# csulb-datascience/TTS-with-Diffusion-model

Measured on AMD Instinct MI355X. Metric: EnCodec codec-tokens/sec (whole node), 100-step D3PM, higher is better.
Workload: dtype bf16; 1 GPU; libritts: d=512 H=8 L=6 T=750/768 S_text=50 S_prompt=225 99 diffusion iterations, n_q=1; utterances_per_gpu=32, global_batch=32, parallelism=dp1, streams_per_gpu=1

## Files before the change

tts-with-diffusion-model_amd/csrc/d3pm_api.hip:

```cpp
#include <cmath>
#include <cstdarg>
#include <cstdio>
#include <new>
#include <vector>

#include "d3pm_plan.h"

namespace d3pm {

static thread_local char g_err[512] = "";
void set_error(const char* fmt, ...) {
  va_list ap;
  va_start(ap, fmt);
  vsnprintf(g_err, sizeof(g_err), fmt, ap);
  va_end(ap);
}

int q_sample_launch(const d3pm_shape*, int, const int32_t*, int32_t*, const uint8_t*, int, const d3pm_schedule*,
                    uint64_t, uint32_t, hipStream_t);
int uniform_launch(uint64_t, int, uint32_t, int, int, int, float*, hipStream_t);
int ce_loss_launch(int, const void*, int, const int32_t*, const uint8_t*, int, int, int, float*, hipStream_t);
float host_h2f(uint16_t h);

}
// ... 940 lines not shown
                      void* workspace, size_t workspace_bytes, void* logits_out, void* hidden_out, int only_layers,
                      uint32_t flags, void* stream) {
  return denoise_step_impl(sh, w, batch, x_t, shared_mask(sh, frame_mask), t, film, kv_text, kv_prompt, workspace, workspace_bytes, logits_out,
                           hidden_out, only_layers, flags, stream, nullptr);
}

int d3pm_denoise_step_canvas(const d3pm_shape* sh, const d3pm_weights* w, int batch, const int32_t* x_t, const d3pm_canvas* canvas, int t,
                             const void* film, const void* kv_text, const void* kv_prompt, void* workspace, size_t workspace_bytes,
                             void* logits_out, void* hidden_out, int only_layers, uint32_t flags, void* stream) {
  D3PM_REQUIRE(canvas, D3PM_E_ARG, "d3pm_denoise_step_canvas: null canvas");
  return denoise_step_impl(sh, w, batch, x_t, per_utterance_mask(sh, batch, canvas, false), t, film, kv_text, kv_prompt, workspace, workspace_bytes,
                           logits_out, hidden_out, only_layers, flags, stream, nullptr);
}

int d3pm_denoise_step_keys(const d3pm_shape* sh, const d3pm_weights* w, int batch, const int32_t* x_t, const d3pm_canvas* canvas, int t,
                           const void* film, const void* kv_text, const void* kv_prompt, void* workspace, size_t workspace_bytes,
                           void* logits_out, void* hidden_out, int only_layers, uint32_t flags, const d3pm_keys* keys, void* stream) {
  D3PM_REQUIRE(canvas, D3PM_E_ARG, "d3pm_denoise_step_keys: null canvas");
  return denoise_step_impl(sh, w, batch, x_t, per_utterance_mask(sh, batch, canvas, false), t, film, kv_text, kv_prompt, workspace, workspace_bytes,
                           logits_out, hidden_out, only_layers, flags, stream, nullptr, key_counts(keys));
}

int d3pm_denoise_step_fp8(const d3pm_shape* sh, const d3pm_weights* w, const d3pm_fp8_block_weights* fp8_blocks, int batch,
                          const int32_t* x_t, const uint8_t* frame_mask, int t, const void* film, const void* kv_text,
                          const void* kv_prompt, void* workspace, size_t workspace_bytes, void* logits_out, void* hidden_out,
                          int only_layers, uint32_t flags, void* stream) {
  D3PM_REQUIRE(fp8_blocks, D3PM_E_ARG, "d3pm_denoise_step_fp8: null fp8 weights");
  return denoise_step_impl(sh, w, batch, x_t, shared_mask(sh, frame_mask), t, film, kv_text, kv_prompt, workspace, workspace_bytes, logits_out,
                           hidden_out, only_layers, flags, stream, fp8_blocks);
}

static int check_sampling(const d3pm_shape* sh, const d3pm_nucleus* sm, const char* who) {
  if (!sm) return D3PM_OK;
  D3PM_REQUIRE(std::isfinite(sm->temperature) && sm->temperature > 0.f, D3PM_E_ARG, "%s: temperature %g is not a finite number > 0", who,
               static_cast<double>(sm->temperature));
  D3PM_REQUIRE(sm->top_k >= 0 && sm->top_k <= sh->n_classes, D3PM_E_ARG, "%s: top_k %d outside 0 (off) .. %d (n_classes)", who, sm->top_k,
               sh->n_classes);
  D3PM_REQUIRE(std::isfinite(sm->top_p) && sm->top_p > 0.f && sm->top_p <= 1.f, D3PM_E_ARG, "%s: top_p %g outside (0, 1] (1 = off)", who,
               static_cast<double>(sm->top_p));
  return D3PM_OK;
}
static const d3pm_nucleus* with_top_p_off(const d3pm_sampling* sm, d3pm_nucleus* out) {
  if (!sm) return nullptr;
  *out = d3pm_nucleus{sm->temperature, sm->top_k, 1.0f};
  return out;
}

static int posterior_sample_impl(const d3pm_shape* sh, int batch, const void* logits, int logits_dtype, const int32_t* x_t,
                                 int32_t* x_next, const uint8_t* known, int t, const d3pm_schedule* sched, uint64_t seed, uint32_t utt0,
                                 uint32_t flags, uint16_t* posterior_out, void* stream, const d3pm_nucleus* sm = nullptr,
                                 float* theta_out = nullptr, const char* who = "d3pm_posterior_sample_sampling") {
  D3PM_TRY(check_shape(sh, batch));
  D3PM_TRY(check_sampling(sh, sm, who));
  D3PM_REQUIRE(logits && x_t && x_next && sched && sched->d && sched->c && sched->dbar && sched->cbar, D3PM_E_ARG,
               "d3pm_posterior_sample: null pointer");
  D3PM_REQUIRE(t >= 0 && t < sched->timesteps, D3PM_E_ARG, "t=%d outside the schedule", t);
  SampleArgs a;
  a.logits = logits; a.logits_dtype = logits_dtype; a.ldl = sh->n_classes; a.x_t = x_t; a.x_next = x_next;
  a.posterior_out = posterior_out; a.rows = batch * sh->canvas * levels(*sh); a.n_classes = sh->n_classes; a.mask_id = sh->mask_id;
  a.n_q = levels(*sh);
  a.canvas = sh->canvas; a.seed = seed; a.row0 = utt0 * static_cast<uint32_t>(sh->canvas);
  a.greedy = (flags & D3PM_FLAG_GREEDY) ? 1 : 0; a.pc = make_posterior_consts(sched, t);
  a.known = known;
  if (sm) { a.temperature = sm->temperature; a.top_k = sm->top_k; a.top_p = sm->top_p; }
  a.theta_out = theta_out;
  return posterior_sample(a, static_cast<hipStream_t>(stream));
}

int d3pm_posterior_sample(const d3pm_shape* sh, int batch, const void* logits, int logits_dtype, const int32_t* x_t,
                          int32_t* x_next, int t, const d3pm_schedule* sched, uint64_t seed, uint32_t utt0,
                          uint32_t flags, uint16_t* posterior_out, void* stream) {
  return posterior_sample_impl(sh, batch, logits, logits_dtype, x_t, x_next, nullptr, t, sched, seed, utt0, flags, posterior_out, stream);
}

int d3pm_posterior_sample_known(const d3pm_shape* sh, int batch, const void* logits, int logits_dtype, const int32_t* x_t,
                                int32_t* x_next, const uint8_t* known, int t, const d3pm_schedule* sched, uint64_t seed, uint32_t utt0,
                                uint32_t flags, uint16_t* posterior_out, void* stream) {
  return posterior_sample_impl(sh, batch, logits, logits_dtype, x_t, x_next, known, t, sched, seed, utt0, flags, posterior_out, stream);
}

int d3pm_posterior_sample_sampling(const d3pm_shape* sh, int batch, const void* logits, int logits_dtype, const int32_t* x_t,
                                   int32_t* x_next, const uint8_t* known, int t, const d3pm_schedule* sched, uint64_t seed, uint32_t utt0,
                                   uint32_t flags, uint16_t* posterior_out, const d3pm_sampling* sampling, void* stream) {
  d3pm_nucleus nu;
  return posterior_sample_impl(sh, batch, logits, logits_dtype, x_t, x_next, known, t, sched, seed, utt0, flags, posterior_out, stream,
                               with_top_p_off(sampling, &nu));
}

int d3pm_posterior_sample_nucleus(const d3pm_shape* sh, int batch, const void* logits, int logits_dtype, const int32_t* x_t,
                                  int32_t* x_next, const uint8_t* known, int t, const d3pm_schedule* sched, uint64_t seed, uint32_t utt0,
                                  uint32_t flags, uint16_t* posterior_out, const d3pm_nucleus* nucleus, float* theta_out, void* stream) {
  return posterior_sample_impl(sh, batch, logits, logits_dtype, x_t, x_next, known, t, sched, seed, utt0, flags, posterior_out, stream, nucleus,
                               theta_out, "d3pm_posterior_sample_nucleus");
}

int d3pm_op_posterior_sample_rows(const d3pm_shape* sh, int batch, const void* logits, int logits_dtype, int ldl, const int32_t* row_of,
                                  const int32_t* x_t, int32_t* x_next, int32_t* x_next2, const uint8_t* known, int t,
                                  const d3pm_schedule* sched, uint64_t seed, uint32_t utt0, uint32_t flags, const d3pm_nucleus* nucleus,
                                  const d3pm_guidance* guidance, void* stream) {
  const char* who = "d3pm_op_posterior_sample_rows";
  D3PM_TRY(check_shape(sh, batch));
  D3PM_TRY(check_sampling(sh, nucleus, who));
  D3PM_REQUIRE(logits && x_t && x_next && sched && sched->d && sched->c && sched->dbar && sched->cbar, D3PM_E_ARG, "%s: null pointer", who);
  D3PM_REQUIRE(t >= 0 && t < sched->timesteps, D3PM_E_ARG, "t=%d outside the schedule", t);
  D3PM_REQUIRE(ldl >= sh->n_classes, D3PM_E_ARG, "%s: row stride %d below n_classes %d", who, ldl, sh->n_classes);
  D3PM_REQUIRE(!(flags & D3PM_FLAG_SEED_IN_HBM), D3PM_E_ARG, "%s: the seed travels by value", who);
  SampleArgs a;
  a.logits = logits; a.logits_dtype = logits_dtype; a.ldl = ldl; a.x_t = x_t; a.x_next = x_next; a.x_next2 = x_next2;
  a.rows = batch * sh->canvas * levels(*sh); a.n_classes = sh->n_classes; a.mask_id = sh->mask_id; a.n_q = levels(*sh);
  a.canvas = sh->canvas; a.seed = seed; a.row0 = utt0 * static_cast<uint32_t>(sh->canvas);
  a.greedy = (flags & D3PM_FLAG_GREEDY) ? 1 : 0; a.pc = make_posterior_consts(sched, t);
  a.known = known;
  if (nucleus) { a.temperature = nucleus->temperature; a.top_k = nucleus->top_k; a.top_p = nucleus->top_p; }
  if (guidance) { a.guided = true; a.guidance = guidance->weight; }
  return posterior_sample_dedup(a, row_of, NextIterPrep{}, static_cast<hipStream_t>(stream));
}

static int sample_loop_impl(const d3pm_shape* sh, const d3pm_weights* w, int batch, int32_t* x, const CanvasMask& cm,
                            int t_start, int t_stop, const void* film, const void* kv_text, const void* kv_prompt,
                            const d3pm_schedule* sched, uint64_t seed, uint32_t utt0, uint32_t flags, void* workspace,
                            size_t workspace_bytes, int32_t* trace, void* stream, const d3pm_fp8_block_weights* f8,
                            const d3pm_nucleus* sm = nullptr, const char* who = "d3pm_sample_loop_sampling", const KeyCounts& keys = KeyCounts{},
                            const d3pm_guidance* guide = nullptr) {
  D3PM_TRY(check_shape(sh, batch));
  D3PM_TRY(check_sampling(sh, sm, who));
  D3PM_REQUIRE(w && w->blocks && x && cm.frame_mask && film && kv_text && kv_prompt && sched && workspace, D3PM_E_ARG,
               "d3pm_sample_loop: null pointer");
  D3PM_REQUIRE(t_start < sched->timesteps && t_start <= sh->timesteps && t_stop >= 0 && t_stop <= t_start, D3PM_E_ARG,
               "bad step range %d..%d", t_start, t_stop);
  d3pm_shape gsh;
  d3pm_tuning gtune;
  if (guide) {
    gtune = tune_of(sh->tuning);
    gtune.regime_batch = 2 * (gtune.regime_batch > batch ? gtune.regime_batch : batch);
    gsh = *sh;
    gsh.tuning = &gtune;
    sh = &gsh;
  }
  const int eval_batch = guide ? 2 * batch : batch;
  Workspace ws = carve(*sh, eval_batch, static_cast<char*>(workspace));
  D3PM_REQUIRE(workspace_bytes >= ws.total, D3PM_E_WORKSPACE, "workspace %zu < required %zu", workspace_bytes, ws.total);
  hipStream_t s = static_cast<hipStream_t>(stream);
  const int rows = batch * sh->canvas;
  const Ctx cx(sh->tuning);
  DenoiserArgs q{*sh, *w, eval_batch, cm.frame_mask, cm.period, kv_text, kv_prompt, ws, keys, guide ? rows : 0};
  const int plan = fold_plan(q, flags, f8);
  if (plan != FOLD_NONE && tune_of(sh->tuning).ln_fold != 2 && levels(*sh) == 1 && !guide && t_start - t_stop >= 2 && ws.tab_qkv) {
    D3PM_TRY(build_qkv_table(cx, *sh, *w, ws, s));
    q.qkv_table = ws.tab_qkv;
  }
  const int n_rows = eval_batch * sh->canvas;
  const int ln_fold = tune_of(sh->tuning).ln_fold;
  if (q.qkv_table && plan == FOLD_QUADS && (ln_fold == 1 || ln_fold == 4) && !f8 && !guide && ws.dd.row_of && n_rows % 384 == 0 && sh->n_layers <= 16 &&
      sh->n_classes <= kDedupMaxClasses && ws.h2 == at(ws.h, static_cast<size_t>(n_rows) * sh->d_model, dtype_size(sh->dtype))) {
    DedupPlanner dp{sh->dtype, sh->tuning, true};
    for (int l = 0; l < sh->n_layers; ++l) (void)folded_block(q, l, true, dp, l == 0);
    LinearArgs fin = projection(ws.x, w->final_w, w->final_b, ws.logits, n_rows, sh->n_classes, sh->d_model);
    fin.ldy = logits_ld(*sh); fin.tune = sh->tuning;
    const LinearPlan fp = plan_linear(sh->dtype, fin);
    const unsigned long long kv_rows = std::max<unsigned long long>(n_rows, qkv_table_rows(sh->n_classes));
    const bool gather_ok = static_cast<size_t>(sh->canvas) * 4 <= kGatherIndexBytes && kv_rows * 3 * sh->d_model * dtype_size(sh->dtype) < (1ull << 32);
    if (dp.ok && gather_ok && (fp.big() || fp.kernel == LIN_128_GLDS)) q.dd = &ws.dd;
  }
  bool latency_ok = false;
  if (q.dd && ln_fold == 1 && !cm.known) {
    DenoiserArgs ql = q;
    ql.m_est = live_latency_rows();
    DedupPlanner lp{sh->dtype, sh->tuning, true, LIN_PANEL64};
    for (int l = 0; l < sh->n_layers; ++l) (void)folded_block(ql, l, false, lp, l == 0);
    latency_ok = lp.ok;
  }
  auto latency_est = [&](int t) {
    if (!latency_ok || t <= t_stop) return 0;
    const int est = plan_live_rows(eval_batch, sh->canvas, host_h2f(sched->cbar[t]));
    return live_latency(est) ? est : 0;
  };
  bool prepared = false;
  bool qkv_ready = false;
  for (int t = t_start; t > t_stop; --t) {
    if (cx.prof) cx.prof->sample_now = (t % cx.prof->stride) == 0;
    q.m_est = latency_est(t);
    D3PM_TRY(denoiser_blocks(q, x, t, film, sh->n_layers, flags, s, f8, q.m_est ? FOLD_PARTS : plan, prepared, qkv_ready));
    prepared = qkv_ready = false;
    SampleArgs a;
    a.logits = ws.logits; a.logits_dtype = sh->dtype; a.ldl = logits_ld(*sh); a.x_t = x; a.x_next = x;
    a.x_next2 = trace ? trace + static_cast<size_t>(t_start - t) * rows * levels(*sh) : nullptr;
    a.rows = rows * levels(*sh); a.n_q = levels(*sh); a.n_classes = sh->n_classes; a.mask_id = sh->mask_id; a.canvas = sh->canvas; a.seed = seed;
    if (flags & D3PM_FLAG_SEED_IN_HBM) a.seed_hbm = reinterpret_cast<const uint64_t*>(static_cast<uintptr_t>(seed));
    a.row0 = utt0 * static_cast<uint32_t>(sh->canvas); a.greedy = (flags & D3PM_FLAG_GREEDY) ? 1 : 0;
    a.pc = make_posterior_consts(sched, t);
    a.known = cm.known;
    if (sm) { a.temperature = sm->temperature; a.top_k = sm->top_k; a.top_p = sm->top_p; }
    if (guide) { a.guided = true; a.guidance = guide->weight; }
    {
      D3PM_TRY(final_logits(*sh, *w, eval_batch, ws, ws.logits, logits_ld(*sh), flags, s, q.dd ? q.dd->m_live : nullptr));
      const bool preps = t - 1 > t_stop && plan != FOLD_NONE;
      if (q.dd) {
        NextIterPrep nx;
        if (preps) {
          nx.dtype = sh->dtype; nx.d = sh->d_model; nx.blocks = w->blocks; nx.n_layers = sh->n_layers;
          nx.film_t = at(film, static_cast<size_t>(t - 1) * sh->n_layers * 2 * sh->d_model, dtype_size(sh->dtype));
          nx.Wf = ws.fc1f; nx.s_out = ws.fc1f_s; nx.b_out = ws.fc1f_b;
        }
        {
          ProfScope p(cx, D3PM_K_SAMPLE, s, 0.0, static_cast<double>(rows) * (sh->n_classes * dtype_size(sh->dtype) + 8.0));
          D3PM_TRY(posterior_sample_dedup(a, q.dd->row_of, nx, s));
        }
        if (preps) {
          D3PM_TRY(run_dedup_index(q, x, plan == FOLD_QUADS && !latency_est(t - 1), s));
          prepared = qkv_ready = true;
        }
        continue;
      }
      ProfScope p(cx, D3PM_K_SAMPLE, s, 0.0,
                  static_cast<double>(rows) * levels(*sh) * ((guide ? 2.0 : 1.0) * sh->n_classes * dtype_size(sh->dtype) + 8.0) +
                      (preps && q.qkv_table ? static_cast<double>(rows) * 3.0 * sh->d_model * dtype_size(sh->dtype) : 0.0));
      NextIterPrep nx;
      if (preps) {
        const size_t es = dtype_size(sh->dtype);
        nx.dtype = sh->dtype; nx.table = w->resps_emb; nx.x = ws.x; nx.stats = ws.stats; nx.frame_mask = cm.frame_mask; nx.mask_period = cm.period; nx.d = sh->d_model;
        nx.quads = plan == FOLD_QUADS;
        nx.blocks = w->blocks; nx.n_layers = sh->n_layers;
        nx.film_t = at(film, static_cast<size_t>(t - 1) * sh->n_layers * 2 * sh->d_model, es);
        nx.Wf = ws.fc1f; nx.s_out = ws.fc1f_s; nx.b_out = ws.fc1f_b;
        if (q.qkv_table) { nx.qkv_table = q.qkv_table; nx.q0 = ws.q0; nx.kv0 = ws.kv0; }
      }
      if (nx.table && posterior_sample_prep_supported(a, nx)) {
        D3PM_TRY(guide ? posterior_sample_prep_guided(a, nx, s) : posterior_sample_prep(a, nx, s));
        prepared = true;
        qkv_ready = nx.q0 != nullptr;
      } else {
        D3PM_TRY(guide ? posterior_sample_guided(a, s) : posterior_sample(a, s));
      }
    }
  }
  if (cx.prof) cx.prof->sample_now = false;
  return D3PM_OK;
}

int d3pm_sample_loop(const d3pm_shape* sh, const d3pm_weights* w, int batch, int32_t* x, const uint8_t* frame_mask,
                     int t_start, int t_stop, const void* film, const void* kv_text, const void* kv_prompt,
                     const d3pm_schedule* sched, uint64_t seed, uint32_t utt0, uint32_t flags, void* workspace,
                     size_t workspace_bytes, int32_t* trace, void* stream) {
  return sample_loop_impl(sh, w, batch, x, shared_mask(sh, frame_mask), t_start, t_stop, film, kv_text, kv_prompt, sched, seed, utt0, flags,
                          workspace, workspace_bytes, trace, stream, nullptr);
}

int d3pm_sample_loop_canvas(const d3pm_shape* sh, const d3pm_weights* w, int batch, int32_t* x, const d3pm_canvas* canvas,
                            int t_start, int t_stop, const void* film, const void* kv_text, const void* kv_prompt,
                            const d3pm_schedule* sched, uint64_t seed, uint32_t utt0, uint32_t flags, void* workspace,
                            size_t workspace_bytes, int32_t* trace, void* stream) {
  D3PM_REQUIRE(canvas, D3PM_E_ARG, "d3pm_sample_loop_canvas: null canvas");
  return sample_loop_impl(sh, w, batch, x, per_utterance_mask(sh, batch, canvas, true), t_start, t_stop, film, kv_text, kv_prompt, sched, seed,
                          utt0, flags, workspace, workspace_bytes, trace, stream, nullptr);
}

int d3pm_sample_loop_fp8(const d3pm_shape* sh, const d3pm_weights* w, const d3pm_fp8_block_weights* fp8_blocks, int batch,
                         int32_t* x, const uint8_t* frame_mask, int t_start, int t_stop, const void* film,
                         const void* kv_text, const void* kv_prompt, const d3pm_schedule* sched, uint64_t seed, uint32_t utt0,
                         uint32_t flags, void* workspace, size_t workspace_bytes, int32_t* trace, void* stream) {
  D3PM_REQUIRE(fp8_blocks, D3PM_E_ARG, "d3pm_sample_loop_fp8: null fp8 weights");
  return sample_loop_impl(sh, w, batch, x, shared_mask(sh, frame_mask), t_start, t_stop, film, kv_text, kv_prompt, sched, seed, utt0, flags,
                          workspace, workspace_bytes, trace, stream, fp8_blocks);
}

int d3pm_sample_loop_fp8_canvas(const d3pm_shape* sh, const d3pm_weights* w, const d3pm_fp8_block_weights* fp8_blocks, int batch,
                                int32_t* x, const d3pm_canvas* canvas, int t_start, int t_stop, const void* film,
                                const void* kv_text, const void* kv_prompt, const d3pm_schedule* sched, uint64_t seed, uint32_t utt0,
                                uint32_t flags, void* workspace, size_t workspace_bytes, int32_t* trace, void* stream) {
  D3PM_REQUIRE(fp8_blocks && canvas, D3PM_E_ARG, "d3pm_sample_loop_fp8_canvas: null fp8 weights or canvas");
  return sample_loop_impl(sh, w, batch, x, per_utterance_mask(sh, batch, canvas, true), t_start, t_stop, film, kv_text, kv_prompt, sched, seed,
                          utt0, flags, workspace, workspace_bytes, trace, stream, fp8_blocks);
}

int d3pm_sample_loop_sampling(const d3pm_shape* sh, const d3pm_weights* w, const d3pm_fp8_block_weights* fp8_blocks, int batch, int32_t* x,
                              const uint8_t* frame_mask, const d3pm_canvas* canvas, int t_start, int t_stop, const void* film,
                              const void* kv_text, const void* kv_prompt, const d3pm_schedule* sched, uint64_t seed, uint32_t utt0,
                              uint32_t flags, void* workspace, size_t workspace_bytes, int32_t* trace, const d3pm_sampling* sampling,
                              void* stream) {
  D3PM_REQUIRE(sh && (frame_mask != nullptr) != (canvas != nullptr), D3PM_E_ARG,
               "d3pm_sample_loop_sampling: give exactly one of frame_mask (shared by the batch) and canvas (per utterance)");
  d3pm_nucleus nu;
  return sample_loop_impl(sh, w, batch, x, canvas ? per_utterance_mask(sh, batch, canvas, true) : shared_mask(sh, frame_mask), t_start, t_stop,
                          film, kv_text, kv_prompt, sched, seed, utt0, flags, workspace, workspace_bytes, trace, stream, fp8_blocks,
                          with_top_p_off(sampling, &nu));
}

int d3pm_sample_loop_nucleus(const d3pm_shape* sh, const d3pm_weights* w, const d3pm_fp8_block_weights* fp8_blocks, int batch, int32_t* x,
                             const uint8_t* frame_mask, const d3pm_canvas* canvas, int t_start, int t_stop, const void* film,
                             const void* kv_text, const void* kv_prompt, const d3pm_schedule* sched, uint64_t seed, uint32_t utt0,
                             uint32_t flags, void* workspace, size_t workspace_bytes, int32_t* trace, const d3pm_nucleus* nucleus,
                             void* stream) {
  D3PM_REQUIRE(sh && (frame_mask != nullptr) != (canvas != nullptr), D3PM_E_ARG,
               "d3pm_sample_loop_nucleus: give exactly one of frame_mask (shared by the batch) and canvas (per utterance)");
  return sample_loop_impl(sh, w, batch, x, canvas ? per_utterance_mask(sh, batch, canvas, true) : shared_mask(sh, frame_mask), t_start, t_stop,
                          film, kv_text, kv_prompt, sched, seed, utt0, flags, workspace, workspace_bytes, trace, stream, fp8_blocks, nucleus,
                          "d3pm_sample_loop_nucleus");
}

int d3pm_sample_loop_keys(const d3pm_shape* sh, const d3pm_weights* w, const d3pm_fp8_block_weights* fp8_blocks, int batch, int32_t* x,
                          const uint8_t* frame_mask, const d3pm_canvas* canvas, int t_start, int t_stop, const void* film,
                          const void* kv_text, const void* kv_prompt, const d3pm_schedule* sched, uint64_t seed, uint32_t utt0,
                          uint32_t flags, void* workspace, size_t workspace_bytes, int32_t* trace, const d3pm_nucleus* nucleus,
                          const d3pm_keys* keys, void* stream) {
  D3PM_REQUIRE(sh && (frame_mask != nullptr) != (canvas != nullptr), D3PM_E_ARG,
               "d3pm_sample_loop_keys: give exactly one of frame_mask (shared by the batch) and canvas (per utterance)");
  D3PM_REQUIRE(!(keys && fp8_blocks), D3PM_E_ARG, "d3pm_sample_loop_keys: the fp8 fast path takes no key mask");
// ... 552 lines not shown
```

tts-with-diffusion-model_amd/csrc/d3pm_dedup.hip:

```cpp
#include <climits>

#include "d3pm_kernels.h"
#include "d3pm_fold_rows.h"

namespace d3pm {
namespace {

__device__ __forceinline__ int clamp_id(int id, int n_classes) { return id < 0 ? 0 : (id >= n_classes ? n_classes - 1 : id); }

__global__ __launch_bounds__(256) void dedup_index_utt(const int32_t* __restrict__ tokens, const uint8_t* __restrict__ frame_mask, int mask_period,
                                                       int canvas, int n_classes, int32_t* __restrict__ cnt, int32_t* __restrict__ row_of,
                                                       int32_t* __restrict__ rep_pos, int32_t* __restrict__ key_cls) {
  extern __shared__ int dedup_sm[];
  int* first = dedup_sm;
  int* rank = first + n_classes + 1;
  int* wsum = rank + n_classes + 1;
  const int b = blockIdx.x, tid = threadIdx.x, lane = tid & 63, wave = tid >> 6;
  const size_t row0 = static_cast<size_t>(b) * canvas;
  for (int c = tid; c <= n_classes; c += 256) first[c] = INT_MAX;
  __syncthreads();
  auto class_of = [&](int j) {
    const size_t r = row0 + j;
    return frame_mask[r % mask_period] ? clamp_id(tokens[r], n_classes) : n_classes;
  };
  for (int j = tid; j < canvas; j += 256) atomicMin(&first[class_of(j)], j);
  __syncthreads();
  int base = 0;
  for (int j0 = 0; j0 < canvas; j0 += 256) {
    const int j = j0 + tid;
    int c = 0;
    bool rep = false;
    if (j < canvas) { c = class_of(j); rep = first[c] == j; }
    const unsigned long long m = __ballot(rep);
    if (lane == 0) wsum[wave] = __popcll(m);
    __syncthreads();
    int off = base;
    for (int w = 0; w < wave; ++w) off += wsum[w];
    if (rep) {
      const int k = off + __popcll(m & ((1ull << lane) - 1ull));
      rank[c] = k;
      rep_pos[row0 + k] = j;
    }
    base += wsum[0] + wsum[1] + wsum[2] + wsum[3];
    __syncthreads();
  }
  for (int j = tid; j < canvas; j += 256) {
    const int c = class_of(j);
    row_of[row0 + j] = rank[c];
    if (key_cls) key_cls[row0 + j] = c;
  }
  if (tid == 0) cnt[b] = base;
}

template <typename T>
__global__ __launch_bounds__(256) void dedup_embed_rows(const int32_t* __restrict__ tokens, const uint8_t* __restrict__ frame_mask, int mask_period,
                                                        int batch, int canvas, int n_classes, int d, int seg_align, const int32_t* __restrict__ cnt,
                                                        int32_t* __restrict__ seg_start, int32_t* __restrict__ seg_len, int32_t* __restrict__ m_live_out,
                                                        int32_t* __restrict__ row_of, const int32_t* __restrict__ rep_pos, int32_t* __restrict__ cid,
                                                        uint8_t* __restrict__ cmask, const T* __restrict__ table, T* __restrict__ x,
                                                        float* __restrict__ stats, bool quads, const T* __restrict__ qkv_table, T* __restrict__ q0,
                                                        T* __restrict__ zero0, T* __restrict__ zero1) {
  const int wave = threadIdx.x >> 6, lane = threadIdx.x & 63;
  const int n = batch * canvas;
  const int r = blockIdx.x * 4 + wave;
  if (r >= n) return;
  const int ub = r / canvas;
  int start = 0, u = -1, u_start = 0, u_cnt = 0, pos_start = 0, own_start = 0, own_len = 0;
  for (int b = 0; b < batch; ++b) {
    const int c = cnt[b], pad = (c + seg_align - 1) & ~(seg_align - 1);
    if (r >= start && r < start + pad) { u = b; u_start = start; u_cnt = c; }
    if (b == ub) pos_start = start;
    if (b == r) { own_start = start; own_len = pad; }
    start += pad;
  }
  const int m_live = start, m_pad = (m_live + 383) / 384 * 384;
  if (lane == 0) {
    if (r < batch) { seg_start[r] = own_start; seg_len[r] = own_len; }
    if (r == 0) *m_live_out = m_live;
  }
  if (lane == 0) row_of[r] += pos_start;
  if (r >= m_pad) return;
  int id = 0;
  bool live = false;
  if (u >= 0 && r - u_start < u_cnt) {
    const size_t row = static_cast<size_t>(u) * canvas + rep_pos[static_cast<size_t>(u) * canvas + (r - u_start)];
    id = clamp_id(tokens[row], n_classes);
    live = frame_mask[row % mask_period] != 0;
  }
  if (table) embed_row_stats<T>(table, id, live, x, r, d, n_classes, stats, quads, lane);
  if (qkv_table) {
    const Vec8<T>* ts = reinterpret_cast<const Vec8<T>*>(qkv_table + static_cast<size_t>(live ? id : n_classes) * 3 * d);
    Vec8<T>* tq = reinterpret_cast<Vec8<T>*>(q0 + static_cast<size_t>(r) * d);
    for (int c = lane; c < (d >> 3); c += kWave) tq[c] = ts[c];
  }
  if (lane == 0) {
    cid[r] = live ? id : n_classes;
    cmask[r] = live ? 1 : 0;
  }
  if (r >= m_live) {
    if (zero0) { Vec8<T>* z = reinterpret_cast<Vec8<T>*>(zero0 + static_cast<size_t>(r) * d); for (int c = lane; c < (d >> 3); c += kWave) z[c] = Vec8<T>{}; }
    if (zero1) { Vec8<T>* z = reinterpret_cast<Vec8<T>*>(zero1 + static_cast<size_t>(r) * d); for (int c = lane; c < (d >> 3); c += kWave) z[c] = Vec8<T>{}; }
  }
}

}

int dedup_index(int dtype, const DedupArgs& a, hipStream_t s) {
  const DedupIndex& ix = a.ix;
  D3PM_REQUIRE(a.tokens && a.frame_mask && a.mask_period > 0 && a.batch > 0 && a.canvas > 0 && a.n_classes > 0 && ix.cnt && ix.seg_start && ix.seg_len &&
                   ix.m_live && ix.row_of && ix.rep_pos && ix.cid && ix.cmask,
               D3PM_E_ARG, "row deduplication: null pointer");
  D3PM_REQUIRE(a.seg_align == 1 || a.seg_align == 128, D3PM_E_ARG, "row deduplication: seg_align is 1 or 128, not %d", a.seg_align);
  D3PM_REQUIRE(a.n_classes <= kDedupMaxClasses && a.canvas % 128 == 0 && (static_cast<long long>(a.batch) * a.canvas) % 384 == 0, D3PM_E_SHAPE,
               "row deduplication: at most %d classes, canvas a multiple of 128 and batch * canvas a multiple of 384", kDedupMaxClasses);
  D3PM_REQUIRE((dtype == D3PM_F16 || dtype == D3PM_BF16) && a.d % 8 == 0 && (!a.quads || a.d == 512) && (!a.table || (a.x && a.stats)) &&
                   (a.qkv_table != nullptr) == (a.q0 != nullptr),
               D3PM_E_ARG, "row deduplication: bad embedding arguments");
  const int n = a.batch * a.canvas;
  const size_t lds = (2 * static_cast<size_t>(a.n_classes + 1) + 4) * sizeof(int);
  dedup_index_utt<<<dim3(a.batch), dim3(256), lds, s>>>(a.tokens, a.frame_mask, a.mask_period, a.canvas, a.n_classes, ix.cnt, ix.row_of, ix.rep_pos, ix.key_cls);
  D3PM_LAUNCH_CHECK();
  const dim3 grid(static_cast<unsigned>((n + 3) / 4)), block(256);
  auto go = [&](auto* tag) {
    using U = std::remove_pointer_t<decltype(tag)>;
    dedup_embed_rows<U><<<grid, block, 0, s>>>(a.tokens, a.frame_mask, a.mask_period, a.batch, a.canvas, a.n_classes, a.d, a.seg_align, ix.cnt, ix.seg_start,
                                               ix.seg_len, ix.m_live, ix.row_of, ix.rep_pos, ix.cid, ix.cmask, static_cast<const U*>(a.table), static_cast<U*>(a.x),
                                               a.stats, a.quads, static_cast<const U*>(a.qkv_table), static_cast<U*>(a.q0),
                                               static_cast<U*>(a.zero[0]), static_cast<U*>(a.zero[1]));
  };
  if (dtype == D3PM_F16) go(static_cast<f16*>(nullptr)); else go(static_cast<bf16*>(nullptr));
  D3PM_LAUNCH_CHECK();
  return D3PM_OK;
}

}
```

tts-with-diffusion-model_amd/csrc/d3pm_kernels.h:

```cpp
#pragma once
#include "d3pm_common.h"

namespace d3pm {

enum { ACT_NONE = 0, ACT_GELU = 1, ACT_RELU = 2, ACT_SILU = 3 };

inline const d3pm_tuning& tune_of(const d3pm_tuning* t) {
  static const d3pm_tuning kDefault = { 0,  1024,  0,  0,
                                        1,  1,  10,  1,
                                        0,  1,  nullptr};
  return t ? *t : kDefault;
}

struct LinearArgs {
  const void* X = nullptr; int ldx = 0;
  const void* W = nullptr;
  const void* bias = nullptr;
  void* Y = nullptr; int ldy = 0;
  const void* R1 = nullptr; const void* R2 = nullptr; int ldr = 0;
  const uint8_t* row_mask = nullptr; int mask_period = 1;
  int M = 0, N = 0, K = 0;
  int act = ACT_NONE;
  const d3pm_tuning* tune = nullptr;
  const float* fold_s = nullptr; const float* fold_b = nullptr; const float* stats_in = nullptr; float fold_eps = 1e-6f;
  float* stats_out = nullptr;
  bool moment_quads = false;
  const int* m_live = nullptr;
  int m_est = 0;
};
inline bool fold_args_ok(const LinearArgs& a) {
  auto al16 = [](const void* p) { return (reinterpret_cast<uintptr_t>(p) % 16) == 0; };
  if (a.fold_s) {
    if (!a.fold_b || !a.stats_in || a.R1 || a.row_mask || a.stats_out || (a.act != ACT_NONE && a.act != ACT_GELU)) return false;
    if (a.K % 256 != 0 || a.N % 4 != 0 || !al16(a.fold_s) || !al16(a.fold_b) || !al16(a.stats_in)) return false;
  } else if (a.fold_b || a.stats_in) {
    return false;
  }
  if (a.stats_out) {
    if (!a.R1 || a.act != ACT_NONE || a.N % 32 != 0 || (reinterpret_cast<uintptr_t>(a.stats_out) % 8) != 0) return false;
  }
  if (a.moment_quads) {
    if (!a.fold_s && !a.stats_out) return false;
    if ((a.fold_s && a.K != 512) || (a.stats_out && a.N != 512)) return false;
  }
  return true;
}

struct AttnArgs {
  const void* Q = nullptr; int ldq = 0;
  const void* K = nullptr; const void* V = nullptr; int ldkv = 0;
  void* O = nullptr; int ldo = 0;
  int B = 0, Tq = 0, S = 0, H = 0, hd = 0;
  float scale = 1.f;
  const int32_t* key_len = nullptr;
  const void* Q2 = nullptr; const void* K2 = nullptr; const void* V2 = nullptr; void* O2 = nullptr; int S2 = 0;
  const int32_t* key_len2 = nullptr;
  bool masked_keeps_schedule = false;
  const int32_t* seg_start = nullptr; const int32_t* seg_len = nullptr;
  const int32_t* key_row = nullptr; int kv_rows = 0;
  const d3pm_tuning* tune = nullptr;
};

struct LayerNormArgs {
  const void* X = nullptr; void* Y = nullptr;
  const void* w = nullptr; const void* b = nullptr;
  const void* w2 = nullptr; const void* b2 = nullptr; void* Y2 = nullptr;
  const void* film = nullptr;
  int M = 0, d = 0; float eps = 1e-6f;
  const int32_t* tokens = nullptr; const uint8_t* frame_mask = nullptr; int mask_period = 0, n_classes = 0; void* Xout = nullptr;
};

struct RowPanelFuse {
  const void* X2 = nullptr;
  const void* lnw = nullptr; const void* lnb = nullptr; void* lny = nullptr;
  const void* lnw2 = nullptr; const void* lnb2 = nullptr; void* lny2 = nullptr;
  const void* film = nullptr;
  float eps = 1e-6f;
  void* sx = nullptr; void* sx2 = nullptr;
};

struct EmbedArgs {
  const int32_t* tokens = nullptr; const uint8_t* frame_mask = nullptr; int mask_period = 0;
  const void* table = nullptr; void* Y = nullptr; int M = 0, d = 0, n_classes = 0;
  int n_q = 1;
  const void* qkv_table = nullptr; void* q0 = nullptr; void* kv0 = nullptr;
};
inline int qkv_table_rows(int n_classes) { return (n_classes + 1 + 383) / 384 * 384; }

struct PosteriorConsts {
  float log_f1_zero;
  float log_f1_d;
  float log_f1_c;
  float log_f1_one;
  float dbar_prev;
  float cbar_prev;
  int t;
};

struct SampleArgs {
  const void* logits = nullptr; int logits_dtype = D3PM_F16; int ldl = 0;
  const int32_t* x_t = nullptr; int32_t* x_next = nullptr; int32_t* x_next2 = nullptr;
  uint16_t* posterior_out = nullptr;
  int rows = 0, n_classes = 0, mask_id = 0, canvas = 0;
  uint64_t seed = 0; uint32_t row0 = 0; int greedy = 0;
  const uint64_t* seed_hbm = nullptr;
  int n_q = 1;
  const uint8_t* known = nullptr;
  float temperature = 1.0f; int top_k = 0;
  bool filtered() const { return temperature != 1.0f || top_k != 0; }
  float top_p = 1.0f; float* theta_out = nullptr;
  bool nucleus() const { return top_p < 1.0f || theta_out != nullptr; }
  bool guided = false; float guidance = 0.f;
  PosteriorConsts pc{};
};

int generic_linear(int dtype, const LinearArgs& a, hipStream_t s);
int generic_attention(int dtype, const AttnArgs& a, hipStream_t s);
struct DropoutArgs {
  float p = 0.f, s = 1.f;
  uint64_t seed = 0;
  uint32_t utt0 = 0, site = 0;
};
int generic_attention_dropout_f32(const AttnArgs& a, const DropoutArgs& dr, hipStream_t s);
int generic_layernorm(int dtype, const LayerNormArgs& a, hipStream_t s);
int embed_tokens(int dtype, const EmbedArgs& a, hipStream_t s);
int pad_heads(const void* in, void* out, long long rows, int groups, int hd, hipStream_t s);
int unpad_heads(const void* in, void* out, long long rows, int groups, int hd, hipStream_t s);
int cond_embed_text(int dtype, const int32_t* tok, const void* table, const void* pe0, void* y, int rows, int s_text, int d,
                    int n_classes, const int32_t* key_len, hipStream_t s);
int cond_embed_prompt(int dtype, const int32_t* codes, int n_levels, const void* tables, const void* pe, void* y,
                      int rows, int s_prompt, int d, int n_classes, const int32_t* key_len, hipStream_t s);
int posterior_sample(const SampleArgs& a, hipStream_t s);
struct NextIterPrep {
  int dtype = D3PM_BF16;
  const void* table = nullptr; void* x = nullptr; float* stats = nullptr; const uint8_t* frame_mask = nullptr; int d = 0;
  int mask_period = 0;
  bool quads = false;
  const d3pm_block_weights* blocks = nullptr; int n_layers = 0; const void* film_t = nullptr;
  void* Wf = nullptr; float* s_out = nullptr; float* b_out = nullptr;
  const void* qkv_table = nullptr; void* q0 = nullptr; void* kv0 = nullptr;
};
bool posterior_sample_prep_supported(const SampleArgs& a, const NextIterPrep& n);
int posterior_sample_prep(const SampleArgs& a, const NextIterPrep& n, hipStream_t s);
int posterior_sample_guided(const SampleArgs& a, hipStream_t s);

struct DedupIndex {
  int32_t* cnt = nullptr;
  int32_t* seg_start = nullptr;
  int32_t* seg_len = nullptr;
  int32_t* m_live = nullptr;
  int32_t* row_of = nullptr;
  int32_t* key_cls = nullptr;
  int32_t* rep_pos = nullptr;
  int32_t* cid = nullptr;
  uint8_t* cmask = nullptr;
};
struct DedupArgs {
  const int32_t* tokens = nullptr; const uint8_t* frame_mask = nullptr; int mask_period = 0;
  int batch = 0, canvas = 0, n_classes = 0, d = 0;
  DedupIndex ix;
  int seg_align = 128;
  const void* table = nullptr; void* x = nullptr; float* stats = nullptr; bool quads = false;
  const void* qkv_table = nullptr; void* q0 = nullptr;
  void* zero[2] = {nullptr, nullptr};
};
constexpr int kDedupMaxClasses = 4095;
int dedup_index(int dtype, const DedupArgs& a, hipStream_t s);
int posterior_sample_dedup(const SampleArgs& a, const int32_t* row_of, const NextIterPrep& n, hipStream_t s);
int posterior_sample_prep_guided(const SampleArgs& a, const NextIterPrep& n, hipStream_t s);

struct RevealArgs {
  const void* logits = nullptr; int logits_dtype = D3PM_F16; int ldl = 0;
  const int32_t* x_t = nullptr; int32_t* x_next = nullptr; int32_t* x_next2 = nullptr;
  const uint8_t* frame_mask = nullptr; int mask_period = 0;
  const uint8_t* known = nullptr;
  int32_t* cand = nullptr; float* score = nullptr;
  int rows = 0, canvas = 0, n_classes = 0, mask_id = 0;
  uint64_t seed = 0; uint32_t row0 = 0; int greedy = 0;
  int t = 0;
  float lambda = 0.f;
  float keep_frac = 0.f;
  float temperature = 1.0f; int top_k = 0; float top_p = 1.0f;
  bool filtered() const { return temperature != 1.0f || top_k != 0 || top_p < 1.0f; }
};
int reveal_candidates(const RevealArgs& a, hipStream_t s);
int reveal_commit(const RevealArgs& a, hipStream_t s);
bool reveal_commit_prep_supported(const RevealArgs& a, const NextIterPrep& n);
int reveal_commit_prep(const RevealArgs& a, const NextIterPrep& n, hipStream_t s);

struct MxLinearArgs {
  const void* X8 = nullptr; int ldx = 0; const void* SX = nullptr;
  const void* W8 = nullptr; const void* SW = nullptr;
  const void* bias = nullptr;
  void* Y = nullptr; int ldy = 0;
  const void* R1 = nullptr; int ldr = 0;
  const uint8_t* row_mask = nullptr; int mask_period = 1;
  void* Y8 = nullptr; void* SY = nullptr;
  int M = 0, N = 0, K = 0;
  int act = ACT_NONE;
  const d3pm_tuning* tune = nullptr;
};
bool mx_linear_supported(int dtype, const MxLinearArgs& a);
int mx_linear(int dtype, const MxLinearArgs& a, hipStream_t s);
int layernorm_mx(int dtype, const void* x, uint8_t* y8, uint8_t* sx, const void* w, const void* b, const void* film,
                 const void* w2, const void* b2, uint8_t* y8_2, uint8_t* sx_2, int M, int d, float eps, hipStream_t s);
int quantize_mx(int dtype, const void* x, int ldx, uint8_t* y8, uint8_t* sx, int M, int K, hipStream_t s);

struct LinearPlan;
struct AttnPlan;
int mfma_linear(int dtype, const LinearArgs& a, const LinearPlan& p, hipStream_t s);
int big_linear(int dtype, const LinearArgs& a, const LinearPlan& p, hipStream_t s);
int panel64_linear(int dtype, const LinearArgs& a, const LinearPlan& p, hipStream_t s);
int mfma_attention(int dtype, const AttnArgs& a, const AttnPlan& p, hipStream_t s);
int mfma_attention32(int dtype, const AttnArgs& a, const AttnPlan& p, hipStream_t s);
int mfma_attention32_cross(int dtype, const AttnArgs& a, const AttnPlan& p, hipStream_t s);
int mfma_attention_split(int dtype, const AttnArgs& a, const AttnPlan& p, hipStream_t s);
int panel64_dual(int dtype, const LinearArgs& a, const void* X2, const LinearPlan& p, hipStream_t s);
int big_dual(int dtype, const LinearArgs& a, const void* X2, const LinearPlan& p, hipStream_t s);
bool row_panel_supported(int dtype, const LinearArgs& a, const RowPanelFuse& f);
int row_panel_linear(int dtype, const LinearArgs& a, const RowPanelFuse& f, hipStream_t s);
bool fast_layernorm_supported(int dtype, const LayerNormArgs& a);
int fast_layernorm(int dtype, const LayerNormArgs& a, hipStream_t s);

PosteriorConsts make_posterior_consts(const d3pm_schedule* sched, int t);

bool fold_shape_ok(int dtype, int d);
int fold_rows_launch(int dtype, const void* W, const void* bias, const void* gamma, const void* beta, const void* film, long film_ld,
                     int n_rows, int n_t, int K, void* Wf, float* s_out, float* b_out, hipStream_t s);
int fold_fc1_step_launch(int dtype, const d3pm_block_weights* blocks, int n_layers, const void* film_t, int d, void* Wf, float* s_out,
                         float* b_out, hipStream_t s);
int row_stats_launch(int dtype, const void* x, int ldx, int M, int d, float* stats, hipStream_t s, bool quads = false);
int embed_tokens_stats(int dtype, const EmbedArgs& a, float* stats, bool quads, hipStream_t s);
int qkv_table_rows_launch(int dtype, const void* table, void* x, float* stats, int rows, int d, int n_classes, hipStream_t s);

struct NarEmbedArgs {
  const int32_t* lens = nullptr;
  const int32_t* text = nullptr; int tt_max = 0;
  const int32_t* prom = nullptr; int tp_max = 0; int n_prom_levels = 8;
  const int32_t* resp = nullptr; int tr_max = 0; int resp_stride = 8; int n_given = 1;
  const void *w_text = nullptr, *w_prom = nullptr, *w_resp = nullptr, *sep = nullptr, *pe = nullptr;
  void* x = nullptr; uint8_t* row_mask = nullptr; int32_t* key_len = nullptr;
  int batch = 0, t_max = 0, d = 0, n_tokens = 0;
};
int nar_embed(int dtype, const NarEmbedArgs& a, hipStream_t s);
int adaln(int dtype, const void* x, void* y, const void* emb_row, const uint8_t* row_mask, int M, int d, hipStream_t s);
int nar_sample(int dtype, const void* logits, int ldl, const int32_t* lens, int32_t* resp, int tr_max, int resp_stride,
               int t_max, int n_tokens, int level, float temperature, uint64_t seed, uint32_t utt0, int greedy, int batch,
               hipStream_t s);

}
```

Baseline: 204,600 codec_tokens/s.

## Compute dedup segment offsets once per block via scan and use persistent grid

The dedup embedding kernel used to loop over every utterance in each wave to find segment starts, one wave per row. It now computes the padded segment prefix sums once per block into LDS with a wave-shuffle scan, finds each row's utterance by binary search, and runs a fixed grid of 4 blocks per CU that loops over rows. This removes the redundant per-row O(batch) scan. In exchange it adds an LDS footprint that scales with batch, so a max-batch limit is enforced and the host plan falls back when eval_batch exceeds it.

```diff
diff --git a/tts-with-diffusion-model_amd/csrc/d3pm_api.hip b/tts-with-diffusion-model_amd/csrc/d3pm_api.hip
--- a/tts-with-diffusion-model_amd/csrc/d3pm_api.hip
+++ b/tts-with-diffusion-model_amd/csrc/d3pm_api.hip
@@ -1116,7 +1116,7 @@
   const int n_rows = eval_batch * sh->canvas;
   const int ln_fold = tune_of(sh->tuning).ln_fold;
   if (q.qkv_table && plan == FOLD_QUADS && (ln_fold == 1 || ln_fold == 4) && !f8 && !guide && ws.dd.row_of && n_rows % 384 == 0 && sh->n_layers <= 16 &&
-      sh->n_classes <= kDedupMaxClasses && ws.h2 == at(ws.h, static_cast<size_t>(n_rows) * sh->d_model, dtype_size(sh->dtype))) {
+      sh->n_classes <= kDedupMaxClasses && eval_batch <= kDedupMaxBatch && ws.h2 == at(ws.h, static_cast<size_t>(n_rows) * sh->d_model, dtype_size(sh->dtype))) {
     DedupPlanner dp{sh->dtype, sh->tuning, true};
     for (int l = 0; l < sh->n_layers; ++l) (void)folded_block(q, l, true, dp, l == 0);
     LinearArgs fin = projection(ws.x, w->final_w, w->final_b, ws.logits, n_rows, sh->n_classes, sh->d_model);
diff --git a/tts-with-diffusion-model_amd/csrc/d3pm_dedup.hip b/tts-with-diffusion-model_amd/csrc/d3pm_dedup.hip
--- a/tts-with-diffusion-model_amd/csrc/d3pm_dedup.hip
+++ b/tts-with-diffusion-model_amd/csrc/d3pm_dedup.hip
@@ -2,6 +2,7 @@
 
 #include "d3pm_kernels.h"
 #include "d3pm_fold_rows.h"
+#include "d3pm_plan.h"
 
 namespace d3pm {
 namespace {
@@ -52,6 +53,8 @@
   if (tid == 0) cnt[b] = base;
 }
 
+constexpr int kEmbedGrid = 4 * kCUs;
+
 template <typename T>
 __global__ __launch_bounds__(256) void dedup_embed_rows(const int32_t* __restrict__ tokens, const uint8_t* __restrict__ frame_mask, int mask_period,
                                                         int batch, int canvas, int n_classes, int d, int seg_align, const int32_t* __restrict__ cnt,
@@ -60,46 +63,72 @@
                                                         uint8_t* __restrict__ cmask, const T* __restrict__ table, T* __restrict__ x,
                                                         float* __restrict__ stats, bool quads, const T* __restrict__ qkv_table, T* __restrict__ q0,
                                                         T* __restrict__ zero0, T* __restrict__ zero1) {
-  const int wave = threadIdx.x >> 6, lane = threadIdx.x & 63;
+  extern __shared__ int embed_sm[];
+  int* start = embed_sm;
+  int* wsum = start + batch + 1;
+  const int tid = threadIdx.x, wave = tid >> 6, lane = tid & 63;
   const int n = batch * canvas;
-  const int r = blockIdx.x * 4 + wave;
-  if (r >= n) return;
-  const int ub = r / canvas;
-  int start = 0, u = -1, u_start = 0, u_cnt = 0, pos_start = 0, own_start = 0, own_len = 0;
-  for (int b = 0; b < batch; ++b) {
-    const int c = cnt[b], pad = (c + seg_align - 1) & ~(seg_align - 1);
-    if (r >= start && r < start + pad) { u = b; u_start = start; u_cnt = c; }
-    if (b == ub) pos_start = start;
-    if (b == r) { own_start = start; own_len = pad; }
-    start += pad;
+  int base = 0;
+  for (int b0 = 0; b0 < batch; b0 += 256) {
+    const int b = b0 + tid;
+    const int pad = b < batch ? (cnt[b] + seg_align - 1) & ~(seg_align - 1) : 0;
+    int v = pad;
+#pragma unroll
+    for (int off = 1; off < kWave; off <<= 1) {
+      const int o = __shfl_up(v, off, kWave);
+      if (lane >= off) v += o;
+    }
+    if (lane == kWave - 1) wsum[wave] = v;
+    __syncthreads();
+    int before = base;
+    for (int w = 0; w < wave; ++w) before += wsum[w];
+    if (b < batch) start[b] = before + v - pad;
+    base += wsum[0] + wsum[1] + wsum[2] + wsum[3];
+    __syncthreads();
   }
-  const int m_live = start, m_pad = (m_live + 383) / 384 * 384;
-  if (lane == 0) {
-    if (r < batch) { seg_start[r] = own_start; seg_len[r] = own_len; }
-    if (r == 0) *m_live_out = m_live;
+  if (tid == 0) start[batch] = base;
+  __syncthreads();
+  const int m_live = base, m_pad = (m_live + 383) / 384 * 384;
+  if (blockIdx.x == 0) {
+    for (int b = tid; b < batch; b += 256) { seg_start[b] = start[b]; seg_len[b] = start[b + 1] - start[b]; }
+    if (tid == 0) *m_live_out = m_live;
   }
-  if (lane == 0) row_of[r] += pos_start;
-  if (r >= m_pad) return;
-  int id = 0;
-  bool live = false;
-  if (u >= 0 && r - u_start < u_cnt) {
-    const size_t row = static_cast<size_t>(u) * canvas + rep_pos[static_cast<size_t>(u) * canvas + (r - u_start)];
-    id = clamp_id(tokens[row], n_classes);
-    live = frame_mask[row % mask_period] != 0;
+  const int gw = blockIdx.x * 4 + wave, waves = gridDim.x * 4;
+  for (int r0 = gw * kWave; r0 < n; r0 += waves * kWave) {
+    const int r = r0 + lane;
+    if (r < n) row_of[r] += start[r / canvas];
   }
-  if (table) embed_row_stats<T>(table, id, live, x, r, d, n_classes, stats, quads, lane);
-  if (qkv_table) {
-    const Vec8<T>* ts = reinterpret_cast<const Vec8<T>*>(qkv_table + static_cast<size_t>(live ? id : n_classes) * 3 * d);
-    Vec8<T>* tq = reinterpret_cast<Vec8<T>*>(q0 + static_cast<size_t>(r) * d);
-    for (int c = lane; c < (d >> 3); c += kWave) tq[c] = ts[c];
-  }
-  if (lane == 0) {
-    cid[r] = live ? id : n_classes;
-    cmask[r] = live ? 1 : 0;
-  }
-  if (r >= m_live) {
-    if (zero0) { Vec8<T>* z = reinterpret_cast<Vec8<T>*>(zero0 + static_cast<size_t>(r) * d); for (int c = lane; c < (d >> 3); c += kWave) z[c] = Vec8<T>{}; }
-    if (zero1) { Vec8<T>* z = reinterpret_cast<Vec8<T>*>(zero1 + static_cast<size_t>(r) * d); for (int c = lane; c < (d >> 3); c += kWave) z[c] = Vec8<T>{}; }
+  const int m_end = m_pad < n ? m_pad : n;
+  for (int r = gw; r < m_end; r += waves) {
+    int id = 0;
+    bool live = false;
+    if (r < m_live) {
+      int lo = 0, hi = batch - 1;
+      while (lo < hi) {
+        const int mid = (lo + hi + 1) >> 1;
+        if (start[mid] <= r) lo = mid; else hi = mid - 1;
+      }
+      const int u = lo, k = r - start[u];
+      if (k < cnt[u]) {
+        const size_t row = static_cast<size_t>(u) * canvas + rep_pos[static_cast<size_t>(u) * canvas + k];
+        id = clamp_id(tokens[row], n_classes);
+        live = frame_mask[row % mask_period] != 0;
+      }
+    }
+    if (table) embed_row_stats<T>(table, id, live, x, r, d, n_classes, stats, quads, lane);
+    if (qkv_table) {
+      const Vec8<T>* ts = reinterpret_cast<const Vec8<T>*>(qkv_table + static_cast<size_t>(live ? id : n_classes) * 3 * d);
+      Vec8<T>* tq = reinterpret_cast<Vec8<T>*>(q0 + static_cast<size_t>(r) * d);
+      for (int c = lane; c < (d >> 3); c += kWave) tq[c] = ts[c];
+    }
+    if (lane == 0) {
+      cid[r] = live ? id : n_classes;
+      cmask[r] = live ? 1 : 0;
+    }
+    if (r >= m_live) {
+      if (zero0) { Vec8<T>* z = reinterpret_cast<Vec8<T>*>(zero0 + static_cast<size_t>(r) * d); for (int c = lane; c < (d >> 3); c += kWave) z[c] = Vec8<T>{}; }
+      if (zero1) { Vec8<T>* z = reinterpret_cast<Vec8<T>*>(zero1 + static_cast<size_t>(r) * d); for (int c = lane; c < (d >> 3); c += kWave) z[c] = Vec8<T>{}; }
+    }
   }
 }
 
@@ -116,14 +145,15 @@
   D3PM_REQUIRE((dtype == D3PM_F16 || dtype == D3PM_BF16) && a.d % 8 == 0 && (!a.quads || a.d == 512) && (!a.table || (a.x && a.stats)) &&
                    (a.qkv_table != nullptr) == (a.q0 != nullptr),
                D3PM_E_ARG, "row deduplication: bad embedding arguments");
-  const int n = a.batch * a.canvas;
+  D3PM_REQUIRE(a.batch <= kDedupMaxBatch, D3PM_E_SHAPE, "row deduplication: at most %d utterances", kDedupMaxBatch);
   const size_t lds = (2 * static_cast<size_t>(a.n_classes + 1) + 4) * sizeof(int);
   dedup_index_utt<<<dim3(a.batch), dim3(256), lds, s>>>(a.tokens, a.frame_mask, a.mask_period, a.canvas, a.n_classes, ix.cnt, ix.row_of, ix.rep_pos, ix.key_cls);
   D3PM_LAUNCH_CHECK();
-  const dim3 grid(static_cast<unsigned>((n + 3) / 4)), block(256);
+  const dim3 grid(kEmbedGrid), block(256);
+  const size_t embed_lds = (static_cast<size_t>(a.batch) + 1 + 4) * sizeof(int);
   auto go = [&](auto* tag) {
     using U = std::remove_pointer_t<decltype(tag)>;
-    dedup_embed_rows<U><<<grid, block, 0, s>>>(a.tokens, a.frame_mask, a.mask_period, a.batch, a.canvas, a.n_classes, a.d, a.seg_align, ix.cnt, ix.seg_start,
+    dedup_embed_rows<U><<<grid, block, embed_lds, s>>>(a.tokens, a.frame_mask, a.mask_period, a.batch, a.canvas, a.n_classes, a.d, a.seg_align, ix.cnt, ix.seg_start,
                                                ix.seg_len, ix.m_live, ix.row_of, ix.rep_pos, ix.cid, ix.cmask, static_cast<const U*>(a.table), static_cast<U*>(a.x),
                                                a.stats, a.quads, static_cast<const U*>(a.qkv_table), static_cast<U*>(a.q0),
                                                static_cast<U*>(a.zero[0]), static_cast<U*>(a.zero[1]));
diff --git a/tts-with-diffusion-model_amd/csrc/d3pm_kernels.h b/tts-with-diffusion-model_amd/csrc/d3pm_kernels.h
--- a/tts-with-diffusion-model_amd/csrc/d3pm_kernels.h
+++ b/tts-with-diffusion-model_amd/csrc/d3pm_kernels.h
@@ -165,6 +165,7 @@
   void* zero[2] = {nullptr, nullptr};
 };
 constexpr int kDedupMaxClasses = 4095;
+constexpr int kDedupMaxBatch = 12 * 1024 - 5;
 int dedup_index(int dtype, const DedupArgs& a, hipStream_t s);
 int posterior_sample_dedup(const SampleArgs& a, const int32_t* row_of, const NextIterPrep& n, hipStream_t s);
 int posterior_sample_prep_guided(const SampleArgs& a, const NextIterPrep& n, hipStream_t s);
```

New measurement: 207,700 codec_tokens/s, median of 6. +1.5%, better.
